# achao2013/deep3dmap

Measured on AMD Instinct MI355X. Metric: rendered Mpix/s fwd+bwd, 100k-tri mesh @512x512, higher is better.
Workload: dtype f32

## Files before the change

### deep3dmap_amd/csrc/d3m_edge_grad.h

```cpp
#pragma once
#include <algorithm>
#include <atomic>
#include <type_traits>
#include "d3m_backward.h"
#include "d3m_face_major.h"
#include "d3m_launch.h"

namespace d3m {

#ifndef D3M_EG_INLINE_MAX
#define D3M_EG_INLINE_MAX 6
#endif
constexpr int EG_INLINE_MAX = D3M_EG_INLINE_MAX;
#ifndef D3M_EG_LINE_WAVES
#define D3M_EG_LINE_WAVES 8
#endif
constexpr int EG_LINE_WAVES = D3M_EG_LINE_WAVES;
constexpr int EG_ITEM_DW = 8;

struct EdgeGradArgs {
    const float4* grad;
    const float2* dot;
    const float* go;
    __device__ __forceinline__ size_t pixel(int axis, size_t view_base, int d0, int d1) const {
// ... 533 lines not shown
}
__device__ __forceinline__ int line_first_record(const EdgePlan& w, size_t line) {
    return w.cap_line ? (int)line * w.cap_line : w.line_slice[line].x;
}

constexpr int EG_WINDOW_MAX_S = 2048;
struct LineWindow {
    int* lds;
    int stride;
    __device__ __forceinline__ int* cnt(int axis) const { return lds + axis * stride; }
};
__device__ __forceinline__ void window_open(LineWindow& win, int* lds, int is) {
    win.lds = lds; win.stride = is + 1;
    for (int k = threadIdx.x; k < 2 * (is + 1); k += blockDim.x) lds[k] = 0;
}
__device__ __forceinline__ void window_ranges(const LineWindow& win, const LaneTable& t, int is, bool on, int n_cross, int view,
                                              int* s_lo, int* s_hi) {
    if (threadIdx.x < 2) { s_lo[threadIdx.x] = is; s_hi[threadIdx.x] = -1; }
    __syncthreads();
    const int l = threadIdx.x;
    if (on && n_cross > 0 && (t.bn_axis[l] >> 1) == view) {
        const int axis = t.bn_axis[l] & 1, from = t.d0_from[l], to1 = from + n_cross;
        atomicAdd(&win.cnt(axis)[from], 1);
        atomicAdd(&win.cnt(axis)[to1], -1);
        atomicMin(&s_lo[axis], from);
        atomicMax(&s_hi[axis], to1);
    }
    __syncthreads();
}

template <class FS>
__global__ void __launch_bounds__(256) k_edge_count_window(FS fs, int is, EdgePlan w) {
    extern __shared__ int s_window[];
    __shared__ LaneTable t;
    __shared__ int s_lo[2], s_hi[2];
    LineWindow win;
    window_open(win, s_window, is);
    const int n_blocks = (*w.n_visible + EG_FACES_PER_BLOCK - 1) / EG_FACES_PER_BLOCK;
    const XcdOrder xo(n_blocks);
    const int wv = threadIdx.x >> 6, lane = lane_id();
    for (int i = blockIdx.x; xo.more(i); i += gridDim.x) {
        const int blk = xo.unit(i);
        if (blk >= n_blocks) continue;
        bool on;
        int pos = 0, ea = 0, n_cross = 0;
        const int total = publish_lanes(fs, w.visible_list, w.n_visible, blk, is, t, on, pos, ea, n_cross);
        if (threadIdx.x < EG_FACES_PER_BLOCK * 6 && blk * EG_FACES_PER_BLOCK + (int)threadIdx.x / 6 < *w.n_visible) {
            const size_t lane6 = (size_t)blk * EG_FACES_PER_BLOCK * 6 + threadIdx.x;
            w.lane_cross[lane6] = make_int2(t.pre[threadIdx.x], n_cross);
        }
        if (threadIdx.x == 0) w.lane_block[blk] = total;
        const int view = t.bn_axis[0] >> 1;
        window_ranges(win, t, is, on, n_cross, view, s_lo, s_hi);
        if (wv < 2) {
            const int axis = wv;
            int run = 0;
            for (int d0 = s_lo[axis] + lane; d0 - lane <= s_hi[axis]; d0 += 64) {
                const bool in = d0 <= s_hi[axis];
                const int v = in ? win.cnt(axis)[d0] : 0;
                const int incl = wave_inclusive_scan(v) + run;
                run = __builtin_amdgcn_readlane(incl, 63);
                if (in) {
                    win.cnt(axis)[d0] = 0;
                    if (incl > 0) atomicAdd(&w.line_cursor[((size_t)view * 2 + axis) * is + d0], incl);
                }
            }
        }
        if (on && n_cross > 0 && (t.bn_axis[threadIdx.x] >> 1) != view) {
            const int l = threadIdx.x;
            const size_t line0 = ((size_t)(t.bn_axis[l] >> 1) * 2 + (t.bn_axis[l] & 1)) * is + t.d0_from[l];
            for (int k = 0; k < n_cross; k++) atomicAdd(&w.line_cursor[line0 + k], 1);
        }
        __syncthreads();
    }
}

template <class FS>
__global__ void __launch_bounds__(256) k_edge_count(FS fs, int is, EdgePlan w) {
    __shared__ LaneTable t;
    const int n_blocks = (*w.n_visible + EG_FACES_PER_BLOCK - 1) / EG_FACES_PER_BLOCK;
    const XcdOrder xo(n_blocks);
    for (int i = blockIdx.x; xo.more(i); i += gridDim.x) {
        const int blk = xo.unit(i);
        if (blk >= n_blocks) continue;
        bool on;
        int pos = 0, ea = 0, n_cross = 0;
        const int total = publish_lanes(fs, w.visible_list, w.n_visible, blk, is, t, on, pos, ea, n_cross);
        if (threadIdx.x < EG_FACES_PER_BLOCK * 6 && blk * EG_FACES_PER_BLOCK + (int)threadIdx.x / 6 < *w.n_visible) {
            const size_t lane6 = (size_t)blk * EG_FACES_PER_BLOCK * 6 + threadIdx.x;
            w.lane_cross[lane6] = make_int2(t.pre[threadIdx.x], n_cross);
        }
        if (threadIdx.x == 0) w.lane_block[blk] = total;
        for (int c0 = 0; c0 < total; c0 += 256) {
            const int c = c0 + threadIdx.x;
            size_t line = 0;
            if (c < total) {
                const int l = crossing_lane(t, c);
                line = ((size_t)(t.bn_axis[l] >> 1) * 2 + (t.bn_axis[l] & 1)) * is + t.d0_from[l] + (c - t.pre[l]);
            }
            const unsigned long long same = wave_match_any((uint32_t)line, c < total);
            if (c < total && lane_id() == __builtin_ctzll(same)) atomicAdd(&w.line_cursor[line], __popcll(same));
        }
        __syncthreads();
    }
}

__global__ void __launch_bounds__(256) k_alloc_ranges(const int* __restrict__ counts, int2* __restrict__ line_slice,
                                                     int* __restrict__ cursor, long n) {
    __shared__ int s_wave[4];
    __shared__ int s_base;
    const long i = (long)blockIdx.x * 256 + threadIdx.x;
    const int c = i < n ? counts[i] : 0;
    const int incl = wave_inclusive_scan(c);
    const int lane = lane_id(), wv = threadIdx.x >> 6;
    if (lane == 63) s_wave[wv] = incl;
    __syncthreads();
    if (threadIdx.x == 0) {
        const int t0 = s_wave[0], t1 = s_wave[1], t2 = s_wave[2], t3 = s_wave[3];
        s_base = atomicAdd(cursor, t0 + t1 + t2 + t3);
        s_wave[0] = 0; s_wave[1] = t0; s_wave[2] = t0 + t1; s_wave[3] = t0 + t1 + t2;
    }
    __syncthreads();
    if (i < n) line_slice[i] = make_int2(s_base + s_wave[wv] + incl - c, c);
}

__global__ void __launch_bounds__(256) k_alloc_plan(int* __restrict__ lane_block, const int* __restrict__ n_visible, int per_block,
                                                   int* __restrict__ cursor_a, int blocks_a,
                                                   int* __restrict__ line_count, int2* __restrict__ line_slice,
                                                   int* __restrict__ cursor_b, long n_lines) {
    __shared__ int s_wave[4];
    __shared__ int s_base;
    const bool first = (int)blockIdx.x < blocks_a;
    const long n = first ? (long)((*n_visible + per_block - 1) / per_block) : n_lines;
    const long i = (long)(first ? blockIdx.x : blockIdx.x - blocks_a) * 256 + threadIdx.x;
    if (i - threadIdx.x >= n) return;
    const int c = i < n ? (first ? lane_block[i] : line_count[i]) : 0;
    const int incl = wave_inclusive_scan(c);
    const int lane = lane_id(), wv = threadIdx.x >> 6;
    if (lane == 63) s_wave[wv] = incl;
    __syncthreads();
    if (threadIdx.x == 0) {
        const int t0 = s_wave[0], t1 = s_wave[1], t2 = s_wave[2], t3 = s_wave[3];
        s_base = atomicAdd(first ? cursor_a : cursor_b, t0 + t1 + t2 + t3);
        s_wave[0] = 0; s_wave[1] = t0; s_wave[2] = t0 + t1; s_wave[3] = t0 + t1 + t2;
    }
    __syncthreads();
    if (i < n) {
        const int at = s_base + s_wave[wv] + incl - c;
        if (first) lane_block[i] = at;
        else { line_slice[i] = make_int2(at, c); line_count[i] = 0; }
    }
}

template <class FS, bool ONE_PASS>
__global__ void __launch_bounds__(256) k_edge_scatter(FS fs, const int32_t* __restrict__ face_index_map, int is, EdgePlan w,
                                                     int parts) {
    __shared__ LaneTable t;
    __shared__ float s_slope[3][256];
    __shared__ int s_cbase;
    const int n_blocks = (*w.n_visible + EG_FACES_PER_BLOCK - 1) / EG_FACES_PER_BLOCK;
    const int n_units = n_blocks * parts;
    const XcdOrder xo(n_units);
    for (int i = blockIdx.x; xo.more(i); i += gridDim.x) {
        const int unit = xo.unit(i);
        if (unit >= n_units) continue;
        const int blk = unit / parts, part = unit - blk * parts;
        bool on;
        int pos = 0, ea = 0, n_cross = 0;
        const int total = publish_lanes(fs, w.visible_list, w.n_visible, blk, is, t, on, pos, ea, n_cross);
        if constexpr (ONE_PASS) {
            if (threadIdx.x < EG_FACES_PER_BLOCK * 6 && blk * EG_FACES_PER_BLOCK + (int)threadIdx.x / 6 < *w.n_visible)
                w.lane_cross[(size_t)blk * EG_FACES_PER_BLOCK * 6 + threadIdx.x] = make_int2(t.pre[threadIdx.x], n_cross);
            if (threadIdx.x == 0) {
                const int r = blk % EG_PLAN_CURSORS;
                const long share = w.cap / EG_PLAN_CURSORS;
                const long at = (long)r * share + atomicAdd(&w.alloc[EG_ALLOC_CURSORS + r * EG_CURSOR_STRIDE], total);
                const bool fits = at + total <= (long)(r + 1) * share;
                if (!fits) w.alloc[EG_ALLOC_FULL] = 1;
                else w.lane_block[blk] = (int)at;
                s_cbase = fits ? (int)at : -1;
            }
        }
        {
            const int l = threadIdx.x;
            const EdgeSlopes sl = edge_slopes(t.p[0][l], t.p[1][l], t.p[2][l], t.p[3][l], t.p[4][l], t.p[5][l]);
            s_slope[0][l] = sl.s01; s_slope[1][l] = sl.s02; s_slope[2][l] = sl.s12;
        }
        __syncthreads();
        const long cbase = ONE_PASS ? (long)s_cbase : (long)w.lane_block[blk];
        const bool records = ONE_PASS ? cbase >= 0 : plan_records(w);
        for (int c0 = part * 256; records && c0 < total; c0 += parts * 256) {
            const int c = c0 + threadIdx.x;
            const bool active = c < total;
            int l = 0;
            size_t line = 0;
            int slice_x = 0;
            if (active) {
                l = crossing_lane(t, c);
                line = ((size_t)(t.bn_axis[l] >> 1) * 2 + (t.bn_axis[l] & 1)) * is + t.d0_from[l] + (c - t.pre[l]);
                if (!ONE_PASS) slice_x = w.line_slice[line].x;
            }
            XGeom g;
            bool wants = false;
            if (active) {
                const int bn = t.bn_axis[l] >> 1, axis = t.bn_axis[l] & 1, d0 = t.d0_from[l] + (c - t.pre[l]);
                const int32_t* view = face_index_map + (size_t)bn * is * is;
                g = crossing_geometry(t.p[0][l], t.p[1][l], t.p[2][l], t.p[3][l], t.p[4][l], t.p[5][l],
                                      EdgeSlopes{s_slope[0][l], s_slope[1][l], s_slope[2][l]}, axis, t.fn[l], is, d0,
                                      [&](int e0, int e1) { return view[axis ? (size_t)e0 * is + e1 : (size_t)e1 * is + e0]; });
                wants = (g.bits & XG_ALIVE) && !(g.bits & XG_IDLE);
                if (!wants) w.xpos[cbase + c] = -1;
            }
            const unsigned long long same = wave_match_any((uint32_t)line, wants);
            const int leader = wants ? __builtin_ctzll(same) : 0, n = wants ? __popcll(same) : 0;
            int cursor_base = 0;
            if (wants && lane_id() == leader) cursor_base = atomicAdd(&w.line_cursor[line], n);
            const int in_line = __shfl(cursor_base, leader, 64) + mask_rank(same);
            if (wants) {
                if (ONE_PASS && in_line >= w.cap_line) {
                    w.xpos[cbase + c] = -1;
                    w.alloc[EG_ALLOC_SPILL] = 1;
                } else {
                    const size_t at = ONE_PASS ? line * (size_t)w.cap_line + in_line : (size_t)slice_x + in_line;
                    w.xrec[at] = geometry_to_record(g, t.fn[l]);
                    w.xpos[cbase + c] = (int)at;
                }
            }
        }
        __syncthreads();
    }
}

template <class FS>
__global__ void __launch_bounds__(256) k_edge_overflow(FS fs, EdgeGradArgs a, EdgePlan w, float2* __restrict__ lane_partial) {
    if (plan_complete(w)) return;
    __shared__ LaneTable t;
    __shared__ float4 s_r[256];
    const bool records = plan_records(w);
    const int is = a.S;
    const float two_over_is = 2.0f / (float)is;
    const int n_blocks = (*w.n_visible + EG_FACES_PER_BLOCK - 1) / EG_FACES_PER_BLOCK;
    const XcdOrder xo(n_blocks);
    for (int i = blockIdx.x; xo.more(i); i += gridDim.x) {
        const int blk = xo.unit(i);
        if (blk >= n_blocks) continue;
        bool on;
        int pos = 0, ea = 0, n_cross = 0;
        const int total = publish_lanes(fs, w.visible_list, w.n_visible, blk, is, t, on, pos, ea, n_cross);
        const long cbase = records ? (long)w.lane_block[blk] : 0;
        const int me = threadIdx.x, my_first = t.pre[me], my_end = my_first + n_cross;
        float2 acc = make_float2(0.0f, 0.0f);
        for (int c0 = 0; c0 < total; c0 += 256) {
            const int c = c0 + threadIdx.x;
            float4 r = make_float4(0.0f, 0.0f, 0.0f, 0.0f);
            if (c < total) {
                const int l = crossing_lane(t, c);
                const int d0 = t.d0_from[l] + (c - t.pre[l]);
                const int bn = t.bn_axis[l] >> 1, axis = t.bn_axis[l] & 1, fn = t.fn[l];
                const size_t line = ((size_t)bn * 2 + axis) * is + d0;
                if (!records || line_spilled(w, w.line_cursor[line])) {
                    if (records) w.xpos[cbase + c] = -1;
                    const size_t base = (size_t)bn * is * is;
                    const XGeom xg = crossing_geometry(t.p[0][l], t.p[1][l], t.p[2][l], t.p[3][l], t.p[4][l], t.p[5][l],
                                                       edge_slopes(t.p[0][l], t.p[1][l], t.p[2][l], t.p[3][l], t.p[4][l], t.p[5][l]),
                                                       axis, fn, is, d0,
                                                       [&](int e0, int e1) { return __float_as_int(a.rec_dot(a.pixel(axis, base, e0, e1)).y); });
#pragma unroll
                    for (int which = 0; which < 2; which++) {
                        float g0 = 0, g1 = 0;
                        Segment sg;
                        if (geometry_segment(xg, which, axis, d0, is, a.extent_lo(line), a.extent_hi(line), sg)) {
                            const SegRef ref = load_ref(a, axis, base, sg.d0, sg.ref_pos);
                            walk_inline(a, base, sg, sg.from, sg.to, ref, fn, two_over_is, g0, g1);
                        }
                        if (which == 0) { r.x = g0; r.y = g1; } else { r.z = g0; r.w = g1; }
                    }
                }
            }
            s_r[threadIdx.x] = r;
            __syncthreads();
            for (int k = max(my_first, c0); k < min(my_end, c0 + 256); k++) {
                const float4 q = s_r[k - c0];
                acc.x += q.x; acc.y += q.y;
                acc.x += q.z; acc.y += q.w;
            }
            __syncthreads();
        }
        if (me < EG_FACES_PER_BLOCK * 6 && blk * EG_FACES_PER_BLOCK + me / 6 < *w.n_visible)
            lane_partial[(size_t)blk * EG_FACES_PER_BLOCK * 6 + me] = acc;
        __syncthreads();
    }
}

#ifndef D3M_EG_ROW
#define D3M_EG_ROW 4
#endif
constexpr int EG_ROW = D3M_EG_ROW;
constexpr int EG_SEG_PER_WAVE = 64 / EG_ROW;
constexpr size_t eg_line_static_lds(int waves) { return (size_t)waves * 64 * (EG_ITEM_DW * 4 + 2) + 1024; }
constexpr size_t EG_LINE_STATIC_LDS = eg_line_static_lds(EG_LINE_WAVES);

template <bool USE_RGB, bool USE_ALPHA, int WAVES>
__global__ void __launch_bounds__(WAVES * 64, 8) k_edge_lines(EdgeGradArgs a, EdgePlan w, float2* __restrict__ lane_partial) {
    constexpr int EG_LINE_THREADS = WAVES * 64, EG_QUEUE = EG_LINE_THREADS, EG_LINE_WAVES = WAVES;
    extern __shared__ __attribute__((aligned(16))) float s_line[];
    (void)lane_partial;
    if (!plan_records(w)) return;
    __shared__ __attribute__((aligned(16))) uint32_t s_items[EG_LINE_THREADS * EG_ITEM_DW];
    __shared__ int s_hist[33];
    __shared__ unsigned short s_order[EG_LINE_THREADS];
    __shared__ int s_nitems, s_pass[2];
    constexpr int NZ_CAP = USE_RGB ? 1 : WAVES * 64;
    __shared__ unsigned short s_nz[NZ_CAP];
    __shared__ int s_wcnt[USE_RGB ? 1 : WAVES];
    const int is = a.S;
    auto do_line = [&](const size_t line) {
    const int n_x = __builtin_amdgcn_readfirstlane(line_records(w, line));
    if (n_x <= 0) return;
    const int wv = __builtin_amdgcn_readfirstlane((int)(threadIdx.x >> 6));
    auto lane_here = [] { int t = (int)threadIdx.x; asm volatile("" : "+v"(t)); return t & 63; };
    const int d0 = (int)(line % is);
    const int axis = (int)((line / is) & 1);
    const size_t bn = line / ((size_t)2 * is);
    const size_t view_base = bn * is * is;
    const int x_first = __builtin_amdgcn_readfirstlane(line_first_record(w, line));
    const uint4* xrec = w.xrec + (size_t)x_first;
    const float two_over_is = 2.0f / (float)is;
    const int p_lo = __builtin_amdgcn_readfirstlane(a.extent_lo(line));
    const int p_hi = __builtin_amdgcn_readfirstlane(a.extent_hi(line));
    auto load_record = [&](int ci) {
        uint4 r = make_uint4(0, 0, 0, 0);
        if (ci < n_x) r = xrec[(uint32_t)ci];
        return r;
    };
    float2* s_df = (float2*)s_line;
    float4* s_grd = (float4*)(s_df + is + (is & 1));
    float4* s_val = s_grd + is;
    const float go_sign = a.go_sign();
    constexpr bool VOID_TILES = USE_RGB && USE_ALPHA;
    for (int p = (int)threadIdx.x; p < is; p += EG_LINE_THREADS) {
        const size_t pi = a.pixel(axis, view_base, d0, p);
        float4 v = make_float4(0, 0, 0, 0);
        if (VOID_TILES && a.void_at(bn, axis, d0, p)) {
            v = a.void_value(bn);
        } else {
            if (USE_ALPHA) v.x = a.alpha_map[pi];
            if (USE_RGB) { v.y = a.rgb_map[3 * pi]; v.z = a.rgb_map[3 * pi + 1]; v.w = a.rgb_map[3 * pi + 2]; }
        }
        s_val[p] = v;
    }
    for (int p = p_lo + (int)threadIdx.x; p <= p_hi; p += EG_LINE_THREADS) {
        const size_t pi = a.pixel(axis, view_base, d0, p);
        float4 g;
        float2 d;
        if (VOID_TILES && a.void_at(bn, axis, d0, p)) {
            g = make_float4(0.0f, 0.0f, 0.0f, 0.0f);
            d = make_float2(0.0f, __int_as_float(-1));
        } else if (!USE_RGB && a.direct()) {
            const float ga = a.direct_ga_at(bn, axis, d0, p, pi);
            g = make_float4(ga, 0.0f, 0.0f, 0.0f);
            d = make_float2(a.alpha_map[pi] * ga, __int_as_float(a.fi_direct[pi]));
        } else {
            g = a.grad[pi];
            d = a.dot[pi];
        }
        g.x *= go_sign; g.y *= go_sign; g.z *= go_sign; g.w *= go_sign;
        s_grd[p] = g;
        s_df[p] = make_float2(0.5f * go_sign * d.x, d.y);
    }
    typedef float v2f __attribute__((ext_vector_type(2)));
    auto diff_of = [](const float4 g, const float2 d, const v2f nref_ar, const v2f nref_gb) {
        v2f p = {d.x, d.x};
        p = __builtin_elementwise_fma(v2f{g.x, g.y}, nref_ar, p);
        p = __builtin_elementwise_fma(v2f{g.z, g.w}, nref_gb, p);
        return p.x + p.y;
    };
    auto diff_of2 = [](const float4 g, const float2 d, const v2f nref_ar, const v2f nref_gb) {
        v2f p = {d.x, d.x};
        p = __builtin_elementwise_fma(v2f{g.x, g.y}, nref_ar, p);
        p = __builtin_elementwise_fma(v2f{g.z, g.w}, nref_gb, p);
        return p + __builtin_shufflevector(p, p, 1, 0);
    };
#ifdef D3M_EG_TWO_RCP
    auto rcp2 = [](const v2f den) { return v2f{__builtin_amdgcn_rcpf(den.x), __builtin_amdgcn_rcpf(den.y)}; };
#else
    auto rcp2 = [](const v2f den) {
        const float r = __builtin_amdgcn_rcpf(den.x * den.y);
        return v2f{r, r} * v2f{den.y, den.x};
    };
#endif
    auto fma_where = [](v2f& acc, const v2f d2, const v2f r, const unsigned long long keep) {
#ifdef D3M_EG_SELECT_FMA
        if (__builtin_amdgcn_inverse_ballot_w64(keep)) acc = __builtin_elementwise_fma(d2, r, acc);
#else
        unsigned long long saved;
        asm volatile("s_and_saveexec_b64 %[sv], %[kp]\n\t"
                     "v_pk_fma_f32 %[a], %[d], %[rr], %[a]\n\t"
                     "s_mov_b64 exec, %[sv]"
                     : [a] "+v"(acc), [sv] "=&s"(saved)
                     : [kp] "s"(keep), [d] "v"(d2), [rr] "v"(r)
                     : "scc");
#endif
    };
    auto walk_queue = [&]() {
        const int nc = s_nitems;
        if (nc > 0) {
            int key = -1, rank_in_key = 0;
            if ((int)threadIdx.x < nc) {
                const uint32_t ft = s_items[(size_t)threadIdx.x * EG_ITEM_DW + 2];
                key = 31 - min(((int)(ft >> 16) - (int)(ft & 0xFFFF) + 1) >> 4, 31);
                rank_in_key = atomicAdd(&s_hist[key], 1);
            }
            __syncthreads();
            if (threadIdx.x == 0) {
                int run = 0;
                for (int k = 0; k < 32; k++) { const int c = s_hist[k]; s_hist[k] = run; run += c; }
            }
            __syncthreads();
            if (key >= 0) s_order[s_hist[key] + rank_in_key] = (unsigned short)threadIdx.x;
            __syncthreads();
            constexpr int STRIDE = EG_LINE_WAVES * EG_SEG_PER_WAVE;
            const int row = lane_here() / EG_ROW, rl = lane_here() % EG_ROW;
            for (int base = wv * EG_SEG_PER_WAVE; base < nc; base += STRIDE) {
                const bool have = base + row < nc;
                const int it = have ? s_order[base + row] : s_order[base];
                const uint4* q = (const uint4*)(s_items + (size_t)it * EG_ITEM_DW);
                const uint4 q0v = q[0], q1v = q[1];
                const float4 rv = s_val[q1v.z];
                const uint32_t bits = q0v.x & 63u;
                const int from = (int)(q0v.z & 0xFFFF), to = have ? (int)(q0v.z >> 16) : -1, fn = (int)(q0v.x >> 6);
                const float d1_cross = __uint_as_float(q1v.x);
                const float inv0 = __uint_as_float(q0v.y), inv1 = __uint_as_float(q1v.y);
                const float s_t = (bits & 32u) ? 1.0f : -1.0f;
                const v2f u = {s_t * (a.eps * fabsf(inv0)), s_t * (a.eps * fabsf(inv1))};
                const v2f nref_ar = {USE_ALPHA ? -rv.x : 0.0f, USE_RGB ? -rv.y : 0.0f};
                const v2f nref_gb = {USE_RGB ? -rv.z : 0.0f, USE_RGB ? -rv.w : 0.0f};
                const unsigned long long m_outward = ~__builtin_amdgcn_ballot_w64((bits & 1u) != 0);
                const int len = to - from + 1;
                int max_len = __builtin_amdgcn_readlane(len, 0);
    #pragma unroll
                for (int r = 1; r < EG_SEG_PER_WAVE; r++) max_len = max(max_len, __builtin_amdgcn_readlane(len, r * EG_ROW));
                const int n_iter = (max_len + EG_ROW - 1) / EG_ROW;
                float t = (float)(from + rl) - d1_cross;
                v2f acc = {0.0f, 0.0f};
                {
                    const float4* pg = s_grd + from + rl;
                    const float2* pd = s_df + from + rl;
                    const float4* pg_to = s_grd + to;
                    v2f den = u + t;
                    if (m_outward == ~0ull) {
                        float4 ga = pg[0];
                        float2 da = pd[0];
                        const float4* pg_to1 = pg_to - EG_ROW;
                        for (int k = 0; k < n_iter; k += 2) {
                            const float4 gb = pg[EG_ROW];
                            const float2 db = pd[EG_ROW];
                            {
                                const v2f d2 = diff_of2(ga, da, nref_ar, nref_gb);
                                const unsigned long long keep = __builtin_amdgcn_ballot_w64(pg <= pg_to) &
                                                                __builtin_amdgcn_ballot_w64(!(d2.x <= 0));
                                fma_where(acc, d2, rcp2(den), keep);
                                den += (float)EG_ROW;
                            }
                            ga = pg[2 * EG_ROW];
                            da = pd[2 * EG_ROW];
                            {
                                const v2f d2 = diff_of2(gb, db, nref_ar, nref_gb);
                                const unsigned long long keep = __builtin_amdgcn_ballot_w64(pg <= pg_to1) &
                                                                __builtin_amdgcn_ballot_w64(!(d2.x <= 0));
                                fma_where(acc, d2, rcp2(den), keep);
                                den += (float)EG_ROW;
                            }
                            pg += 2 * EG_ROW;
                            pd += 2 * EG_ROW;
                        }
                    } else {
                        for (int k = 0; k < n_iter; k++) {
                            const float4 g = *pg;
                            const float2 d = *pd;
                            const v2f d2 = diff_of2(g, d, nref_ar, nref_gb);
                            const unsigned long long keep = __builtin_amdgcn_ballot_w64(pg <= pg_to) &
                                                            __builtin_amdgcn_ballot_w64(!(d2.x <= 0)) &
                                                            (__builtin_amdgcn_ballot_w64(__float_as_int(d.y) == fn) | m_outward);
                            const v2f r = rcp2(den);
                            fma_where(acc, d2, r, keep);
                            pg += EG_ROW;
                            pd += EG_ROW;
                            den += (float)EG_ROW;
                        }
                    }
                }
                float s0 = acc.x, s1 = acc.y;
                s0 += dpp_f32<0xB1>(s0);  s1 += dpp_f32<0xB1>(s1);
                s0 += dpp_f32<0x4E>(s0);  s1 += dpp_f32<0x4E>(s1);
                if (EG_ROW >= 8) { s0 += dpp_f32<0x141>(s0); s1 += dpp_f32<0x141>(s1); }
                if (EG_ROW == 16) { s0 += dpp_f32<0x140>(s0); s1 += dpp_f32<0x140>(s1); }
                asm volatile("" ::: "memory");
                if (base + row < nc && rl == 0) {
                    const uint4 z0 = q[0];
                    const uint32_t zbits = z0.x & 63u;
                    const float zinv0 = __uint_as_float(z0.y), zinv1 = __uint_as_float(q[1].y);
                    if (zbits & 24u) {
                        const float4 zrv = s_val[q[1].z];
                        const v2f zref_ar = {USE_ALPHA ? -zrv.x : 0.0f, USE_RGB ? -zrv.y : 0.0f};
                        const v2f zref_gb = {USE_RGB ? -zrv.z : 0.0f, USE_RGB ? -zrv.w : 0.0f};
                        const int df = (zbits & 8u) ? (int)(z0.z & 0xFFFF) : (int)(z0.z >> 16);
                        const float2 d = s_df[df];
                        const float diff = diff_of(s_grd[df], d, zref_ar, zref_gb);
                        const float dpos = (!(diff <= 0) && (!(zbits & 1u) || __float_as_int(d.y) == (int)(z0.x >> 6))) ? diff : 0.0f;
                        const float zs = (zbits & 32u) ? 1.0f : -1.0f;
                        const float ux = zs * (a.eps * fabsf(zinv0)), uy = zs * (a.eps * fabsf(zinv1));
                        if (ux * zinv0 < 0) s0 -= 2.0f * (dpos * __builtin_amdgcn_rcpf(ux));
                        if (uy * zinv1 < 0) s1 -= 2.0f * (dpos * __builtin_amdgcn_rcpf(uy));
                    }
                    w.results[z0.w] = make_float2((zbits & 2u) ? zinv0 * s0 : 0.0f, (zbits & 4u) ? zinv1 * s1 : 0.0f);
                }
            }

        }
        __syncthreads();
        if (threadIdx.x == 0) {
            s_nitems = 0;
#pragma unroll
            for (int k = 0; k < 33; k++) s_hist[k] = 0;
        }
        __syncthreads();
    };
    if (threadIdx.x == 0) {
        s_nitems = 0; s_pass[0] = 0; s_pass[1] = 0;
#pragma unroll
        for (int k = 0; k < 33; k++) s_hist[k] = 0;
    }
    __syncthreads();
    int n_nz = -1;
    if constexpr (!USE_RGB) {
        if (a.sparse_max > 0) {
            const v2f one_ar = {-1.0f, 0.0f}, none_gb = {0.0f, 0.0f};
            int run = 0;
            for (int p0 = p_lo; p0 <= p_hi; p0 += EG_LINE_THREADS) {
                const int p = p0 + (int)threadIdx.x;
                bool on = false;
                if (p <= p_hi) on = !(diff_of(s_grd[p], s_df[p], one_ar, none_gb) <= 0);
                const unsigned long long m = __builtin_amdgcn_ballot_w64(on);
                if (lane_here() == 0) s_wcnt[wv] = __popcll(m);
                __syncthreads();
                int before = run, total = 0;
#pragma unroll
                for (int k = 0; k < WAVES; k++) {
                    const int c = s_wcnt[k];
                    before += k < wv ? c : 0;
                    total += c;
                }
                const int at = before + mask_rank(m);
                if (on && at < NZ_CAP) s_nz[at] = (unsigned short)p;
                run = __builtin_amdgcn_readfirstlane(run + total);
                __syncthreads();
            }
            n_nz = run <= min(a.sparse_max, NZ_CAP) ? run : -1;
        }
    }
    auto make_item = [&](const Segment& q, int fn, uint32_t slot, uint4& rec0, uint4& rec1) {
        const float qc0 = (q.f0 ? q.q0 : 1.0f) * two_over_is, qc1 = (q.f1 ? q.q1 : 1.0f) * two_over_is;
        const float s_t = (float)(q.inward ? -q.dir : q.dir);
        const float rq0 = __builtin_amdgcn_rcpf(qc0), rq1 = __builtin_amdgcn_rcpf(qc1);
        const bool fix = q.inward && (float)q.d1_in == q.d1_cross && q.from <= q.d1_in && q.d1_in <= q.to;
        const uint32_t bits = (uint32_t)q.inward | ((uint32_t)q.f0 << 1) | ((uint32_t)q.f1 << 2) |
                              ((fix && q.dir < 0) ? 8u : 0u) | ((fix && 0 < q.dir) ? 16u : 0u) | (0 < s_t ? 32u : 0u);
        rec0 = make_uint4(bits | ((uint32_t)fn << 6), __float_as_uint(-rq0), (uint32_t)q.from | ((uint32_t)q.to << 16), slot);
        rec1 = make_uint4(__float_as_uint(q.d1_cross), __float_as_uint(-rq1), (uint32_t)q.ref_pos, 0u);
    };
    auto walk_short = [&](const Segment& q, int fn, float& g0, float& g1) {
        const float4 rv = s_val[q.ref_pos];
        const v2f nref_ar = {USE_ALPHA ? -rv.x : 0.0f, USE_RGB ? -rv.y : 0.0f};
        const v2f nref_gb = {USE_RGB ? -rv.z : 0.0f, USE_RGB ? -rv.w : 0.0f};
        const float qq0 = q.f0 ? q.q0 : 1.0f, qq1 = q.f1 ? q.q1 : 1.0f;
        for (int d1 = q.from; d1 <= q.to; d1++) {
            const float2 d = s_df[d1];
            float diff = diff_of(s_grd[d1], d, nref_ar, nref_gb);
            if (q.inward && __float_as_int(d.y) != fn) diff = 0.0f;
            visit_pixel(diff, d1, q.d1_cross, qq0, qq1, q.f0 != 0, q.f1 != 0, two_over_is, a.eps, g0, g1);
        }
    };
    for (int chunk0 = 0, pass = 0, step = EG_LINE_THREADS; chunk0 < n_x; chunk0 += step, pass ^= 1) {
        step = EG_LINE_THREADS;
        const int ci = chunk0 + (int)threadIdx.x;
        unsigned long long qm[2];
        {
            const uint4 rc = load_record(ci);
            const XGeom geo = record_to_geometry(rc);
            const int fn = record_face(rc);
            auto outward = [&]() {
                bool queue_it = false;
                if (ci < n_x) {
                    Segment q;
                    queue_it = geometry_segment(geo, 0, axis, d0, is, p_lo, p_hi, q);
                    float g0 = 0, g1 = 0;
                    if constexpr (!USE_RGB) {
                        if (queue_it && n_nz >= 0 && s_val[q.ref_pos].x == 1.0f) {
                            queue_it = false;
                            int lo = 0, hi = n_nz;
                            while (lo < hi) {
                                const int mid = (lo + hi) >> 1;
                                if ((int)s_nz[mid] < q.from) lo = mid + 1; else hi = mid;
                            }
                            const v2f one_ar = {-1.0f, 0.0f}, none_gb = {0.0f, 0.0f};
                            const float qq0 = q.f0 ? q.q0 : 1.0f, qq1 = q.f1 ? q.q1 : 1.0f;
                            for (int i = lo; i < n_nz; i++) {
                                const int d1 = (int)s_nz[i];
                                if (d1 > q.to) break;
                                visit_pixel_div(diff_of(s_grd[d1], s_df[d1], one_ar, none_gb), d1, q.d1_cross, qq0, qq1, q.f0 != 0,
                                                q.f1 != 0, 2.0f / (float)is, a.eps, g0, g1);
                            }
                        }
                    }
                    if (!queue_it) w.results[2u * (uint32_t)(x_first + ci)] = make_float2(g0, g1);
                }
                qm[0] = __builtin_amdgcn_ballot_w64(queue_it);
            };
            auto inward = [&]() {
                bool queue_it = false;
                if (ci < n_x) {
                    float g0 = 0, g1 = 0;
                    Segment q;
                    if (geometry_segment(geo, 1, axis, d0, is, p_lo, p_hi, q)) {
                        if (segment_queueable(q)) queue_it = true;
                        else walk_short(q, fn, g0, g1);
                    }
                    if (!queue_it) w.results[2u * (uint32_t)(x_first + ci) + 1u] = make_float2(g0, g1);
                }
                qm[1] = __builtin_amdgcn_ballot_w64(queue_it);
            };
            if constexpr (USE_RGB) { outward(); inward(); } else { inward(); outward(); }
        }
        int n0 = __popcll(qm[0]), n1 = __popcll(qm[1]);
        if (lane_here() == 0 && (n0 | n1)) atomicAdd(&s_pass[pass], n0 + n1);
        __syncthreads();
        const int pass_total = s_pass[pass];
        const bool full = s_nitems + pass_total > EG_QUEUE;
        __syncthreads();
        if (full) walk_queue();
        if (threadIdx.x == 0) s_pass[pass ^ 1] = 0;
        if (pass_total > EG_QUEUE) {
            step = EG_LINE_THREADS / 2;
            if ((int)threadIdx.x >= step) { qm[0] = 0; qm[1] = 0; n0 = 0; n1 = 0; }
        }
        if ((qm[0] | qm[1]) != 0) {
            const uint4 rc = load_record(ci);
            const XGeom geo = record_to_geometry(rc);
            const int fn = record_face(rc);
            int base = 0;
            const int lane = lane_here();
            if (lane == 0 && (n0 | n1)) base = atomicAdd(&s_nitems, n0 + n1);
            base = __builtin_amdgcn_readfirstlane(base);
#pragma unroll
            for (int which = 0; which < 2; which++) {
                if ((qm[which] >> lane) & 1ull) {
                    Segment q;
                    geometry_segment(geo, which, axis, d0, is, p_lo, p_hi, q);
                    uint4 rec0, rec1;
                    make_item(q, fn, 2u * (uint32_t)(x_first + ci) + which, rec0, rec1);
                    uint4* it = (uint4*)(s_items + (size_t)(base + (which ? n0 : 0) + mask_rank(qm[which])) * EG_ITEM_DW);
                    it[0] = rec0; it[1] = rec1;
                }
            }
        }
        __syncthreads();
    }
    walk_queue();
    };
    if constexpr (!USE_RGB) {
        if (a.line_left) {
            const int n_left = __builtin_amdgcn_readfirstlane(*a.n_left);
            for (int item = (int)blockIdx.x; item < n_left; item += (int)gridDim.x) {
                do_line((size_t)a.line_left[item]);
                __syncthreads();
            }
            return;
        }
    }
#ifndef D3M_EG_LINES_PLAIN_ORDER
    const XcdOrder xo((int)a.n_lines);
    const size_t line = (size_t)xo.unit((int)blockIdx.x);
    if (line >= a.n_lines) return;
#else
    const size_t line = blockIdx.x;
#endif
    do_line(line);
}

constexpr int EGA_THREADS = 128;
constexpr int EGA_LIST = 128;
inline size_t edge_lines_alpha_lds(int S) { return (size_t)S * 12; }
__global__ void __launch_bounds__(EGA_THREADS) k_edge_lines_alpha(EdgeGradArgs a, EdgePlan w) {
    extern __shared__ __attribute__((aligned(16))) float s_aline[];
    __shared__ unsigned short s_raw[2][EGA_LIST], s_pos[2][EGA_LIST];
    __shared__ int s_n[2], s_odd;
    if (!plan_records(w)) return;
    const int is = a.S;
    const XcdOrder xo((int)a.n_lines);
    const size_t line = (size_t)xo.unit((int)blockIdx.x);
    if (line >= a.n_lines) return;
    const int n_x = __builtin_amdgcn_readfirstlane(line_records(w, line));
    if (n_x <= 0) return;
    const int x_first = __builtin_amdgcn_readfirstlane(line_first_record(w, line));
    const int d0 = (int)(line % is), axis = (int)((line / is) & 1);
    const size_t bn = line / ((size_t)2 * is), view_base = bn * is * is;
    const int p_lo = __builtin_amdgcn_readfirstlane(a.extent_lo(line));
    const int p_hi = __builtin_amdgcn_readfirstlane(a.extent_hi(line));
    float* s_al = s_aline;
    float* s_g = s_al + is;
    int* s_own = (int*)(s_g + is);
    if (threadIdx.x < 2) s_n[threadIdx.x] = 0;
    if (threadIdx.x == 2) s_odd = 0;
    const float go_sign = a.go_sign();
    bool odd = false;
    for (int p0 = (int)threadIdx.x; p0 < is; p0 += 4 * EGA_THREADS) {
        float al[4], gx[4], ow[4];
#pragma unroll
        for (int k = 0; k < 4; k++) {
            const int p = p0 + k * EGA_THREADS;
            const size_t pi = a.pixel(axis, view_base, d0, min(p, is - 1));
            al[k] = a.alpha_map[pi];
            const bool in = p >= p_lo && p <= p_hi;
            gx[k] = in ? (a.direct() ? a.direct_ga_at(bn, axis, d0, min(p, is - 1), pi) : a.grad[pi].x) : 0.0f;
            ow[k] = in ? (a.direct() ? __int_as_float(a.fi_direct[pi]) : a.dot[pi].y) : 0.0f;
        }
#pragma unroll
        for (int k = 0; k < 4; k++) {
            const int p = p0 + k * EGA_THREADS;
            if (p < is) {
                s_al[p] = al[k];
                odd = odd || !(al[k] == 0.0f || al[k] == 1.0f);
                s_g[p] = go_sign * gx[k];
                s_own[p] = __float_as_int(ow[k]);
            }
        }
    }
    __syncthreads();
    if (odd) s_odd = 1;
    for (int p = p_lo + (int)threadIdx.x; p <= p_hi; p += EGA_THREADS) {
        const float al = s_al[p], g = s_g[p];
        if (!((al - 1.0f) * g <= 0)) {
            const int k = atomicAdd(&s_n[0], 1);
            if (k < EGA_LIST) s_raw[0][k] = (unsigned short)p;
        }
        if (!(al * g <= 0)) {
            const int k = atomicAdd(&s_n[1], 1);
            if (k < EGA_LIST) s_raw[1][k] = (unsigned short)p;
        }
    }
    __syncthreads();
    const int n_out = s_n[0], n_in = s_n[1];
    const bool left = n_out > EGA_LIST || n_in > EGA_LIST || s_odd != 0 || a.sparse_max <= 0;
    if (left) {
        if (threadIdx.x == 0) a.line_left[atomicAdd(a.n_left, 1)] = (int)line;
        return;
    }
    for (int e = (int)threadIdx.x; e < n_out + n_in; e += EGA_THREADS) {
        const int which = e < n_out ? 0 : 1, i = which ? e - n_out : e, n = which ? n_in : n_out;
        const unsigned short mine = s_raw[which][i];
        int rank = 0;
        for (int j = 0; j < n; j++) rank += s_raw[which][j] < mine ? 1 : 0;
        s_pos[which][rank] = mine;
    }
    __syncthreads();
    const float two_over_is = 2.0f / (float)is;
    const uint4* xrec = w.xrec + (size_t)x_first;
    uint4 rc_next = make_uint4(0, 0, 0, 0);
    if ((int)threadIdx.x < n_x) rc_next = xrec[threadIdx.x];
    for (int ci = (int)threadIdx.x; ci < n_x; ci += EGA_THREADS) {
        const uint4 rc = rc_next;
        if (ci + EGA_THREADS < n_x) rc_next = xrec[ci + EGA_THREADS];
        const XGeom geo = record_to_geometry(rc);
        const int fn = record_face(rc);
#pragma unroll
        for (int which = 0; which < 2; which++) {
            float g0 = 0.0f, g1 = 0.0f;
            Segment q;
            if (geometry_segment(geo, which, axis, d0, is, p_lo, p_hi, q)) {
                const float ref = s_al[q.ref_pos];
                const int list = ref == 1.0f ? 0 : 1, n = (which == 1 && ref == 1.0f) ? 0 : (list ? n_in : n_out);
                const float qq0 = q.f0 ? q.q0 : 1.0f, qq1 = q.f1 ? q.q1 : 1.0f;
                int lo = 0, hi = n;
                while (lo < hi) {
                    const int mid = (lo + hi) >> 1;
                    if ((int)s_pos[list][mid] < q.from) lo = mid + 1; else hi = mid;
                }
                for (int i = lo; i < n; i++) {
                    const int d1 = (int)s_pos[list][i];
                    if (d1 > q.to) break;
                    if (which == 1 && s_own[d1] != fn) continue;
                    visit_pixel((s_al[d1] - ref) * s_g[d1], d1, q.d1_cross, qq0, qq1, q.f0 != 0, q.f1 != 0, two_over_is, a.eps,
                                g0, g1);
                }
            }
            w.results[2u * (uint32_t)(x_first + ci) + which] = make_float2(g0, g1);
        }
    }
}

constexpr int EG_GATHER_PER = 4;
constexpr int EG_GATHER_CHUNK = 256 * EG_GATHER_PER;
template <class FS>
__global__ void __launch_bounds__(256) k_edge_gather(FS fs, EdgePlan w, const float2* __restrict__ lane_partial,
                                                    const float* __restrict__ go, float* __restrict__ grad_faces,
                                                    VertexTarget vt, int parts) {
    __shared__ float2 s_g[256];
    __shared__ float4 s_res[EG_GATHER_CHUNK];
    __shared__ int s_total;
    if (blockIdx.x == 0 && threadIdx.x == 0) w.alloc[EG_ALLOC_LEFT] = 0;
    const int n_vis = *w.n_visible;
    const int n_blocks = (n_vis + EG_FACES_PER_BLOCK - 1) / EG_FACES_PER_BLOCK;
    const int n_units = n_blocks * parts;
    const XcdOrder xo(n_units);
    const bool records = plan_records(w), complete = plan_complete(w);
    const float go_abs = go ? fabsf(*go) : 1.0f;
    for (int i = blockIdx.x; xo.more(i); i += gridDim.x) {
        const int unit = xo.unit(i);
        if (unit >= n_units) continue;
        const int blk = unit / parts, part = unit - blk * parts;
        const int t = threadIdx.x;
        const int pos = blk * EG_FACES_PER_BLOCK + t / 6, ea = t % 6;
        const bool on = t < EG_FACES_PER_BLOCK * 6 && pos < n_vis;
        float2 g = make_float2(0.0f, 0.0f);
        long gi_top = 0;
        if (parts == 1) {
            const bool use = on && records;
            const int2 lc = use ? w.lane_cross[(size_t)pos * 6 + ea] : make_int2(0, 0);
            const long cb = records ? (long)w.lane_block[blk] : 0;
            if (on && !complete) g = lane_partial[(size_t)pos * 6 + ea];
            if (on && ea == 0) gi_top = w.visible_list[pos];
            if (t == min(EG_FACES_PER_BLOCK, n_vis - blk * EG_FACES_PER_BLOCK) * 6 - 1) s_total = lc.x + lc.y;
            __syncthreads();
            const int total = (int)max(min((long)s_total, (long)w.cap - cb), 0l);
            const int my_end = min(lc.x + lc.y, total);
            const float4* res4 = (const float4*)w.results;
            for (int k0 = 0; k0 < total; k0 += EG_GATHER_CHUNK) {
                int at[EG_GATHER_PER];
#pragma unroll
                for (int j = 0; j < EG_GATHER_PER; j++) {
                    const int k = k0 + j * 256 + t;
                    at[j] = k < total ? w.xpos[cb + k] : -1;
                }
                float4 r[EG_GATHER_PER];
#pragma unroll
                for (int j = 0; j < EG_GATHER_PER; j++)
                    r[j] = at[j] >= 0 ? res4[at[j]] : make_float4(0.0f, 0.0f, 0.0f, 0.0f);
#pragma unroll
                for (int j = 0; j < EG_GATHER_PER; j++) s_res[j * 256 + t] = r[j];
                __syncthreads();
                const int hi = min(my_end, k0 + EG_GATHER_CHUNK);
                for (int k = max(lc.x, k0); k < hi; k += 4) {
                    float4 q[4];
#pragma unroll
                    for (int j = 0; j < 4; j++) q[j] = s_res[min(k + j, hi - 1) - k0];
#pragma unroll
                    for (int j = 0; j < 4; j++) {
                        if (k + j < hi) {
                            g.x += q[j].x; g.y += q[j].y;
                            g.x += q[j].z; g.y += q[j].w;
                        }
                    }
                }
                __syncthreads();
            }
        } else if (on) {
            if (!complete && part == 0) g = lane_partial[(size_t)pos * 6 + ea];
            const int2 lc = records ? w.lane_cross[(size_t)pos * 6 + ea] : make_int2(0, 0);
            const long c_first = records ? (long)w.lane_block[blk] + lc.x : 0, c_last = min(c_first + (long)lc.y, (long)w.cap);
            const float4* res4 = (const float4*)w.results;
            for (long c = c_first + 4 * part; c < c_last; c += 4 * parts) {
                long at[4];
#pragma unroll
                for (int j = 0; j < 4; j++) at[j] = c + j < c_last ? (long)w.xpos[c + j] : -1;
                float4 r[4];
#pragma unroll
                for (int j = 0; j < 4; j++)
                    r[j] = (c + j < c_last && at[j] >= 0) ? res4[at[j]] : make_float4(0.0f, 0.0f, 0.0f, 0.0f);
#pragma unroll
                for (int j = 0; j < 4; j++) {
                    g.x += r[j].x; g.y += r[j].y;
                    g.x += r[j].z; g.y += r[j].w;
                }
            }
        }
        s_g[t] = g;
        __syncthreads();
        if (on && ea == 0) {
            float acc[6] = {0, 0, 0, 0, 0, 0};
#pragma unroll
            for (int e = 0; e < 6; e++) {
                const int edge = e >> 1, axis = e & 1;
                const float2 r = make_float2(s_g[t + e].x * go_abs, s_g[t + e].y * go_abs);
                acc[edge * 2 + (1 - axis)] += r.x;
                acc[((edge + 1) % 3) * 2 + (1 - axis)] += r.y;
            }
            const long gi = parts == 1 ? gi_top : (long)w.visible_list[pos];
            if (vt.gv) {
                const int Fp = fs.num_faces();
                const int b = (int)(gi / Fp), f = (int)(gi % Fp);
#pragma unroll
                for (int v = 0; v < 3; v++) {
                    float* g = vt.vertex(b, f, v);
                    atomicAdd(&g[0], acc[2 * v + 0]);
                    atomicAdd(&g[1], acc[2 * v + 1]);
                }
            } else {
                float* gf = grad_faces + (size_t)gi * 9;
#pragma unroll
                for (int v = 0; v < 3; v++) {
                    gf[3 * v + 0] = acc[2 * v + 0];
                    gf[3 * v + 1] = acc[2 * v + 1];
                    gf[3 * v + 2] = 0.0f;
                }
            }
        }
        __syncthreads();
    }
}

struct ImageGrads {
    const float *g_rgb_out, *g_alpha_out, *g_depth_out;
    float* g_depth_map;
    int s, aa, on;
};
__global__ void __launch_bounds__(256) k_pack_maps(const int32_t* __restrict__ fi, const float* __restrict__ alpha,
                                                  const float* __restrict__ galpha, const float* __restrict__ rgb,
                                                  const float* __restrict__ grgb, float4* __restrict__ grad_row,
                                                  float2* __restrict__ dot_row, int* __restrict__ nz_lo_inv,
                                                  int* __restrict__ nz_hi1, int S, GradScale gs,
                                                  ImageGrads img = ImageGrads{nullptr, nullptr, nullptr, nullptr, 0, 0, 0}) {
    __shared__ int s_col_lo_inv[32], s_col_hi1[32];
    if (threadIdx.x < 32) { s_col_lo_inv[threadIdx.x] = 0; s_col_hi1[threadIdx.x] = 0; }
    __syncthreads();
    const int b = blockIdx.z;
    float s_rgb, s_alpha, s_depth;
    gs.get(s_rgb, s_alpha, s_depth);
    const int x0 = blockIdx.x * 32, y0 = blockIdx.y * 32;
    const int tx = threadIdx.x & 31, ty = threadIdx.x >> 5;
    const size_t plane = (size_t)b * S * S;
    for (int r = ty; r < 32; r += 8) {
        const int y = y0 + r, x = x0 + tx;
        bool nz = false;
        if (y < S && x < S) {
            const size_t i = plane + (size_t)y * S + x;
            float4 g = make_float4(0, 0, 0, 0);
            float dot = 0;
            if (img.on) {
                const int yo = img.aa ? (S - 1 - y) / 2 : S - 1 - y, xo = img.aa ? x / 2 : x;
                const float sc = img.aa ? 0.25f : 1.0f;
                const size_t o = ((size_t)b * img.s + yo) * img.s + xo;
                if (alpha && img.g_alpha_out) { g.x = img.g_alpha_out[o] * sc; dot += alpha[i] * g.x; }
                if (rgb && img.g_rgb_out) {
                    const size_t plane_o = (size_t)img.s * img.s, o0 = ((size_t)b * 3 * img.s + yo) * img.s + xo;
                    g.y = img.g_rgb_out[o0] * sc; g.z = img.g_rgb_out[o0 + plane_o] * sc; g.w = img.g_rgb_out[o0 + 2 * plane_o] * sc;
                    dot += rgb[3 * i] * g.y;
                    dot += rgb[3 * i + 1] * g.z;
                    dot += rgb[3 * i + 2] * g.w;
                }
                if (img.g_depth_map) img.g_depth_map[i] = img.g_depth_out[o] * sc;
            } else if (alpha) { g.x = galpha[i] * s_alpha; dot += alpha[i] * g.x; }
            if (!img.on && rgb) {
                g.y = grgb[3 * i] * s_rgb; g.z = grgb[3 * i + 1] * s_rgb; g.w = grgb[3 * i + 2] * s_rgb;
                dot += rgb[3 * i] * g.y;
                dot += rgb[3 * i + 1] * g.z;
                dot += rgb[3 * i + 2] * g.w;
            }
            const float2 d = make_float2(dot, __int_as_float(fi[i]));
            grad_row[i] = g;
            dot_row[i] = d;
            nz = g.x != 0 || g.y != 0 || g.z != 0 || g.w != 0 || dot != 0;
// ... 337 lines not shown
```

Before: 6013.

## Replace compacted atomic work queue with per-thread fixed slots walked per chunk

The shared work queue for long edge segments is no longer compacted with atomics and ballot ranks. Each thread now writes its queued item straight into its own slot, or marks the slot empty. The queue is then walked once for outward items and once for inward items in every chunk, and the counting sort in walk_queue picks out the valid slots. This removes the atomic base allocation, the overflow and half-step handling, and the rebuild pass. In exchange the queue may be walked up to twice per chunk with partly filled slots and extra barriers, where before it was flushed only when full.

```diff
diff --git a/deep3dmap_amd/csrc/d3m_edge_grad.h b/deep3dmap_amd/csrc/d3m_edge_grad.h
--- a/deep3dmap_amd/csrc/d3m_edge_grad.h
+++ b/deep3dmap_amd/csrc/d3m_edge_grad.h
@@ -859,14 +859,14 @@
 
 template <bool USE_RGB, bool USE_ALPHA, int WAVES>
 __global__ void __launch_bounds__(WAVES * 64, 8) k_edge_lines(EdgeGradArgs a, EdgePlan w, float2* __restrict__ lane_partial) {
-    constexpr int EG_LINE_THREADS = WAVES * 64, EG_QUEUE = EG_LINE_THREADS, EG_LINE_WAVES = WAVES;
+    constexpr int EG_LINE_THREADS = WAVES * 64, EG_LINE_WAVES = WAVES;
     extern __shared__ __attribute__((aligned(16))) float s_line[];
     (void)lane_partial;
     if (!plan_records(w)) return;
     __shared__ __attribute__((aligned(16))) uint32_t s_items[EG_LINE_THREADS * EG_ITEM_DW];
     __shared__ int s_hist[33];
     __shared__ unsigned short s_order[EG_LINE_THREADS];
-    __shared__ int s_nitems, s_pass[2];
+    __shared__ int s_nitems, s_round[2];
     constexpr int NZ_CAP = USE_RGB ? 1 : WAVES * 64;
     __shared__ unsigned short s_nz[NZ_CAP];
     __shared__ int s_wcnt[USE_RGB ? 1 : WAVES];
@@ -959,21 +959,25 @@
                      : "scc");
 #endif
     };
-    auto walk_queue = [&]() {
-        const int nc = s_nitems;
-        if (nc > 0) {
+    auto walk_queue = [&](const int round) {
+        {
             int key = -1, rank_in_key = 0;
-            if ((int)threadIdx.x < nc) {
+            {
                 const uint32_t ft = s_items[(size_t)threadIdx.x * EG_ITEM_DW + 2];
-                key = 31 - min(((int)(ft >> 16) - (int)(ft & 0xFFFF) + 1) >> 4, 31);
-                rank_in_key = atomicAdd(&s_hist[key], 1);
+                const int len = (int)(ft >> 16) - (int)(ft & 0xFFFF) + 1;
+                if (len > 0) {
+                    key = 31 - min(len >> 4, 31);
+                    rank_in_key = atomicAdd(&s_hist[key], 1);
+                }
             }
             __syncthreads();
             if (threadIdx.x == 0) {
                 int run = 0;
                 for (int k = 0; k < 32; k++) { const int c = s_hist[k]; s_hist[k] = run; run += c; }
+                s_nitems = run;
             }
             __syncthreads();
+            const int nc = s_nitems;
             if (key >= 0) s_order[s_hist[key] + rank_in_key] = (unsigned short)threadIdx.x;
             __syncthreads();
             constexpr int STRIDE = EG_LINE_WAVES * EG_SEG_PER_WAVE;
@@ -1077,14 +1081,14 @@
         }
         __syncthreads();
         if (threadIdx.x == 0) {
-            s_nitems = 0;
+            s_round[round] = 0;
 #pragma unroll
             for (int k = 0; k < 33; k++) s_hist[k] = 0;
         }
         __syncthreads();
     };
     if (threadIdx.x == 0) {
-        s_nitems = 0; s_pass[0] = 0; s_pass[1] = 0;
+        s_round[0] = 0; s_round[1] = 0;
 #pragma unroll
         for (int k = 0; k < 33; k++) s_hist[k] = 0;
     }
@@ -1138,10 +1142,11 @@
             visit_pixel(diff, d1, q.d1_cross, qq0, qq1, q.f0 != 0, q.f1 != 0, two_over_is, a.eps, g0, g1);
         }
     };
-    for (int chunk0 = 0, pass = 0, step = EG_LINE_THREADS; chunk0 < n_x; chunk0 += step, pass ^= 1) {
-        step = EG_LINE_THREADS;
+    constexpr uint32_t EG_NO_ITEM = 1u;
+    for (int chunk0 = 0; chunk0 < n_x; chunk0 += EG_LINE_THREADS) {
         const int ci = chunk0 + (int)threadIdx.x;
-        unsigned long long qm[2];
+        uint32_t* const slot = s_items + (size_t)threadIdx.x * EG_ITEM_DW;
+        unsigned long long m_in;
         {
             const uint4 rc = load_record(ci);
             const XGeom geo = record_to_geometry(rc);
@@ -1170,9 +1175,16 @@
                             }
                         }
                     }
-                    if (!queue_it) w.results[2u * (uint32_t)(x_first + ci)] = make_float2(g0, g1);
+                    if (queue_it) {
+                        uint4 rec0, rec1;
+                        make_item(q, fn, 2u * (uint32_t)(x_first + ci), rec0, rec1);
+                        ((uint4*)slot)[0] = rec0; ((uint4*)slot)[1] = rec1;
+                    } else {
+                        w.results[2u * (uint32_t)(x_first + ci)] = make_float2(g0, g1);
+                    }
                 }
-                qm[0] = __builtin_amdgcn_ballot_w64(queue_it);
+                if (!queue_it) slot[2] = EG_NO_ITEM;
+                if (__builtin_amdgcn_ballot_w64(queue_it) != 0 && lane_here() == 0) s_round[0] = 1;
             };
             auto inward = [&]() {
                 bool queue_it = false;
@@ -1185,45 +1197,30 @@
                     }
                     if (!queue_it) w.results[2u * (uint32_t)(x_first + ci) + 1u] = make_float2(g0, g1);
                 }
-                qm[1] = __builtin_amdgcn_ballot_w64(queue_it);
+                m_in = __builtin_amdgcn_ballot_w64(queue_it);
+                if (m_in != 0 && lane_here() == 0) s_round[1] = 1;
             };
             if constexpr (USE_RGB) { outward(); inward(); } else { inward(); outward(); }
         }
-        int n0 = __popcll(qm[0]), n1 = __popcll(qm[1]);
-        if (lane_here() == 0 && (n0 | n1)) atomicAdd(&s_pass[pass], n0 + n1);
         __syncthreads();
-        const int pass_total = s_pass[pass];
-        const bool full = s_nitems + pass_total > EG_QUEUE;
+        if (s_round[0]) walk_queue(0);
+        if (s_round[1]) {
+            bool queue_it = false;
+            if ((m_in >> lane_here()) & 1ull) {
+                const uint4 rc = load_record(ci);
+                const XGeom geo = record_to_geometry(rc);
+                Segment q;
+                queue_it = geometry_segment(geo, 1, axis, d0, is, p_lo, p_hi, q);
+                uint4 rec0, rec1;
+                make_item(q, record_face(rc), 2u * (uint32_t)(x_first + ci) + 1u, rec0, rec1);
+                ((uint4*)slot)[0] = rec0; ((uint4*)slot)[1] = rec1;
+            }
+            if (!queue_it) slot[2] = EG_NO_ITEM;
+            __syncthreads();
+            walk_queue(1);
+        }
         __syncthreads();
-        if (full) walk_queue();
-        if (threadIdx.x == 0) s_pass[pass ^ 1] = 0;
-        if (pass_total > EG_QUEUE) {
-            step = EG_LINE_THREADS / 2;
-            if ((int)threadIdx.x >= step) { qm[0] = 0; qm[1] = 0; n0 = 0; n1 = 0; }
-        }
-        if ((qm[0] | qm[1]) != 0) {
-            const uint4 rc = load_record(ci);
-            const XGeom geo = record_to_geometry(rc);
-            const int fn = record_face(rc);
-            int base = 0;
-            const int lane = lane_here();
-            if (lane == 0 && (n0 | n1)) base = atomicAdd(&s_nitems, n0 + n1);
-            base = __builtin_amdgcn_readfirstlane(base);
-#pragma unroll
-            for (int which = 0; which < 2; which++) {
-                if ((qm[which] >> lane) & 1ull) {
-                    Segment q;
-                    geometry_segment(geo, which, axis, d0, is, p_lo, p_hi, q);
-                    uint4 rec0, rec1;
-                    make_item(q, fn, 2u * (uint32_t)(x_first + ci) + which, rec0, rec1);
-                    uint4* it = (uint4*)(s_items + (size_t)(base + (which ? n0 : 0) + mask_rank(qm[which])) * EG_ITEM_DW);
-                    it[0] = rec0; it[1] = rec1;
-                }
-            }
-        }
-        __syncthreads();
-    }
-    walk_queue();
+    }
     };
     if constexpr (!USE_RGB) {
         if (a.line_left) {
```

After: 6032 (median of 6 runs). No clear change (+0.3%).
